# mushroomfire/mdapy

Hardware: AMD Instinct MI355X
Metric: atoms/sec for neighbor+CNA on 10M-atom FCC Cu; 1/2/4/8-GPU scaling (higher is better)
Workload: dtype f64 (CNA pair tests: f32 filter + f64 finish, labels exact); 1 GPU; FCC Cu a=3.615, 136^3 cells per GPU (10061824 atoms/GPU, 10061824 total), build_neighbor(rc=0.854a=3.08721, max_neigh=16) + fixed-cutoff CNA as one C-ABI call (mdh_build_neighbor_fcna: lists and labels), positions resident in HBM; atoms_per_gpu=10061824, max_neigh=16, parallelism=single, world_size_checked=1, launched_by=single process

## Files before the change

### mdapy_amd/csrc/cna_core.hpp

```cpp
#pragma once
#include "common.hpp"

namespace mdh {

struct Rows {
    uint64_t w0, w1, w2, w3;
    __device__ __forceinline__ unsigned row(int a) const
    {
        const uint64_t w = (a < 8) ? ((a < 4) ? w0 : w1) : ((a < 12) ? w2 : w3);
        return (unsigned)(w >> ((a & 3) << 4)) & 0xffffu;
    }
};

template <int NN>
__device__ __forceinline__ Rows pack_rows(const unsigned (&adj)[NN])
{
    Rows r{0, 0, 0, 0};
#pragma unroll
    for (int a = 0; a < NN; ++a) {
        const uint64_t v = (uint64_t)adj[a] << ((a & 3) << 4);
        if (a < 4) r.w0 |= v;
        else if (a < 8) r.w1 |= v;
        else if (a < 12) r.w2 |= v;
        else r.w3 |= v;
    }
    return r;
}

struct RowsLds {
    const unsigned short *base;
    int stride;
    __device__ __forceinline__ unsigned row(int a) const { return base[a * stride]; }
};
template <int NN>
__device__ __forceinline__ RowsLds spill_rows(const Rows &R, unsigned short *base, int stride)
{
#pragma unroll
    for (int a = 0; a < NN; ++a) base[a * stride] = (unsigned short)R.row(a);
    return RowsLds{base, stride};
}

template <int NN>
struct RowsReg {
    unsigned v[NN];
    __device__ __forceinline__ explicit RowsReg(const unsigned (&adj)[NN])
    {
#pragma unroll
        for (int k = 0; k < NN; ++k) v[k] = adj[k];
    }
    __device__ __forceinline__ unsigned row(int a) const
    {
        unsigned r = v[0];
#pragma unroll
        for (int k = 1; k < NN; ++k) {
            unsigned t = v[k];
            asm("" : "+v"(t));
            r = (a == k) ? t : r;
        }
        return r;
    }
};

template <class RT>
__device__ __forceinline__ void signature(const RT &R, int ni, unsigned limit_mask, int &ncn, int &nb, int &chain)
{
    const unsigned common = R.row(ni);
    ncn = __popc(common);
    const unsigned pool = common & limit_mask;
    int bonds = 0, maxdeg = 0;
    for (unsigned m = pool; m; m &= m - 1) {
        const int deg = __popc(R.row(__ffs(m) - 1) & pool);
        bonds += deg;
        maxdeg = deg > maxdeg ? deg : maxdeg;
    }
    nb = bonds >> 1;
    if (nb <= 1) { chain = nb; return; }
    if (nb == 2) { chain = maxdeg == 2 ? 2 : 1; return; }
    const int npool = __popc(pool);
    if (nb == npool && (npool == 4 || npool == 5)) { chain = nb; return; }
    int best = 0;
    unsigned left = pool;
    while (left) {
        unsigned comp = left & (0u - left), frontier = comp;
        while (frontier) {
            const int a = __ffs(frontier) - 1;
            frontier &= frontier - 1;
            const unsigned grow = R.row(a) & pool & ~comp;
            comp |= grow;
            frontier |= grow;
        }
        int cb = 0;
        for (unsigned m = comp; m; m &= m - 1)
            cb += __popc(R.row(__ffs(m) - 1) & comp);
        cb >>= 1;
        best = cb > best ? cb : best;
        left &= ~comp;
    }
    chain = best;
}

__device__ __forceinline__ double fold(double d, double L, double t_zero, double t_one)
{
    const double shift = (d >= t_one) ? L : ((d >= t_zero) ? 0.0 : -L);
    return d - shift;
}

template <int NN>
__device__ __forceinline__ int span_class(const DBox &b, const double (&p)[NN], int axis)
{
    double mn = p[0], mx = p[0];
#pragma unroll
    for (int a = 1; a < NN; ++a) {
        mn = fmin(mn, p[a]);
        mx = fmax(mx, p[a]);
    }
    const double span = mx - mn;
    const double lim = fmin(b.tn[axis][3], -b.tn[axis][0]);
    const double zero = fmin(b.tn[axis][2], -b.tn[axis][1]);
    if (!(span < lim))
        return 0;
    return span < zero ? 2 : 1;
}

template <bool TRI, int NN>
__device__ __forceinline__ Rows bond_rows_reg(const DBox &b, const double (&px)[NN], const double (&py)[NN],
                                              const double (&pz)[NN], double cut2)
{
    unsigned adj[NN];
#pragma unroll
    for (int a = 0; a < NN; ++a)
        adj[a] = 0;
#pragma unroll
    for (int a = 0; a < NN; ++a)
#pragma unroll
        for (int c = a + 1; c < NN; ++c) {
            const double d2 = pair_d2<TRI>(b, px[a], py[a], pz[a], px[c], py[c], pz[c]);
            if (d2 <= cut2) {
                adj[a] |= 1u << c;
                adj[c] |= 1u << a;
            }
        }
    return pack_rows<NN>(adj);
}

template <int NN>
__device__ __forceinline__ Rows bond_rows_ortho(const DBox &b, const double (&px)[NN], const double (&py)[NN],
                                                const double (&pz)[NN], double cut2, bool plain)
{
    unsigned adj[NN];
#pragma unroll
    for (int a = 0; a < NN; ++a)
        adj[a] = 0;
    if (plain) {
#pragma unroll
        for (int a = 0; a < NN; ++a)
#pragma unroll
            for (int c = a + 1; c < NN; ++c) {
                const double dx = px[c] - px[a], dy = py[c] - py[a], dz = pz[c] - pz[a];
                if (dx * dx + dy * dy + dz * dz <= cut2) {
                    adj[a] |= 1u << c;
                    adj[c] |= 1u << a;
                }
            }
        return pack_rows<NN>(adj);
    }
#pragma unroll
    for (int a = 0; a < NN; ++a)
#pragma unroll
        for (int c = a + 1; c < NN; ++c) {
            double dx = px[c] - px[a], dy = py[c] - py[a], dz = pz[c] - pz[a];
            if (b.pbc[0]) dx = fold(dx, b.h[0], b.tn[0][1], b.tn[0][2]);
            if (b.pbc[1]) dy = fold(dy, b.h[4], b.tn[1][1], b.tn[1][2]);
            if (b.pbc[2]) dz = fold(dz, b.h[8], b.tn[2][1], b.tn[2][2]);
            const double d2 = dx * dx + dy * dy + dz * dz;
            if (d2 <= cut2) {
                adj[a] |= 1u << c;
                adj[c] |= 1u << a;
            }
        }
    return pack_rows<NN>(adj);
}

template <int NN>
__device__ __forceinline__ int span_class3(const DBox &b, const double (&px)[NN], const double (&py)[NN], const double (&pz)[NN])
{
    int cls = 2;
    if (b.pbc[0]) cls = min(cls, span_class<NN>(b, px, 0));
    if (b.pbc[1]) cls = min(cls, span_class<NN>(b, py, 1));
    if (b.pbc[2]) cls = min(cls, span_class<NN>(b, pz, 2));
    return cls;
}

template <int NN, class RT>
__device__ __forceinline__ int fcna_label(const RT &R)
{
    int n421 = 0, n422 = 0, n555 = 0, n444 = 0, n666 = 0;
    for (int ni = 0; ni < NN; ++ni) {
        int ncn, nb, ch;
        signature(R, ni, (1u << NN) - 1u, ncn, nb, ch);
        if (ncn == 4 && nb == 2) { n421 += (ch == 1); n422 += (ch == 2); }
        else if (ncn == 5 && nb == 5 && ch == 5) ++n555;
        else if (ncn == 4 && nb == 4 && ch == 4) ++n444;
        else if (ncn == 6 && nb == 6 && ch == 6) ++n666;
    }
    if (n421 == 12) return 1;
    if (n421 == 6 && n422 == 6) return 2;
    if (n555 == 12) return 4;
    if (n666 == 8 && n444 == 6) return 3;
    return 0;
}

template <int NW>
__device__ __forceinline__ bool six_bonds_one_cluster(const unsigned (&P)[NW], unsigned common, unsigned bonded)
{
    unsigned reach = bonded & (0u - bonded);
#pragma unroll
    for (int it = 0; it < 5; ++it) {
        unsigned acc = 0;
#pragma unroll
        for (int k = 0; k < NW; ++k) {
            const unsigned lo = (unsigned)(((int)(reach << (31 - 2 * k))) >> 31) & 0xffffu;
            const unsigned hi = (unsigned)(((int)(reach << (30 - 2 * k))) >> 31) & 0xffff0000u;
            acc |= P[k] & (lo | hi);
        }
        reach |= (acc | (acc >> 16)) & common & 0xffffu;
    }
    return (bonded & ~reach) == 0u;
}
struct CnaCounts { int n421, n422, n555, n444, n666; };
template <int NN, int MAXO = NN, class RT = RowsLds>
__device__ __forceinline__ CnaCounts cna_counts_words(const unsigned (&adj)[NN], const RT &L)
{
    constexpr int NW = (NN + 1) / 2;
    unsigned P[NW];
#pragma unroll
    for (int k = 0; k < NW; ++k) P[k] = adj[2 * k] | ((2 * k + 1 < NN) ? (adj[2 * k + 1] << 16) : 0u);
    unsigned packed = 0;
#pragma unroll
    for (int ni = 0; ni < NN; ++ni) {
        if (MAXO < NN && (packed >> 20) > (unsigned)MAXO)
            continue;
        const unsigned common = adj[ni];
        const unsigned ncn = (unsigned)__popc(common);
        const unsigned c2 = common | (common << 16);
        unsigned twice = 0, touched = 0;
#pragma unroll
        for (int k = 0; k < NW; ++k) {
            const unsigned lo = (unsigned)(((int)(common << (31 - 2 * k))) >> 31) & 0xffffu;
            const unsigned hi = (unsigned)(((int)(common << (30 - 2 * k))) >> 31) & 0xffff0000u;
            const unsigned xk = P[k] & c2 & (lo | hi);
            twice += __popc(xk);
            touched |= xk;
        }
        const unsigned key = ncn + (twice << 4);
        const unsigned three = (__popc((touched | (touched >> 16)) & 0xffffu) == 3) ? 1u << 4 : 1u;
        unsigned inc = 1u << 20;
        inc = key == 68u ? three : inc;
        inc = key == 165u ? 1u << 8 : inc;
        inc = key == 132u ? 1u << 12 : inc;
        if (key == 198u)
            inc = six_bonds_one_cluster<NW>(P, common, (touched | (touched >> 16)) & 0xffffu) ? 1u << 16 : 1u << 20;
        packed += inc;
    }
    return CnaCounts{(int)(packed & 15u), (int)((packed >> 4) & 15u), (int)((packed >> 8) & 15u), (int)((packed >> 12) & 15u), (int)((packed >> 16) & 15u)};
}
template <int NN, class RT = RowsLds>
__device__ __forceinline__ int fcna_label_words(const unsigned (&adj)[NN], const RT &L)
{
    const CnaCounts c = cna_counts_words<NN, NN - 12, RT>(adj, L);
    if (c.n421 == 12) return 1;
    if (c.n421 == 6 && c.n422 == 6) return 2;
    if (c.n555 == 12) return 4;
    if (c.n666 == 8 && c.n444 == 6) return 3;
    return 0;
}

template <int NN> constexpr int pair_a(int p) { int a = 0; while (p >= NN - 1 - a) { p -= NN - 1 - a; ++a; } return a; }
template <int NN> constexpr int pair_c(int p) { int a = 0; while (p >= NN - 1 - a) { p -= NN - 1 - a; ++a; } return a + 1 + p; }
template <int NN, int NV, int P>
__device__ __forceinline__ void pair_tests_f32(const float (&ux)[NV], const float (&uy)[NV], const float (&uz)[NV], float negc,
                                               unsigned (&adj)[NN], unsigned &w)
{
    constexpr int NP = NN * (NN - 1) / 2;
    if constexpr (P + 1 < NP) {
        constexpr int a0 = pair_a<NN>(P), c0 = pair_c<NN>(P), a1 = pair_a<NN>(P + 1), c1 = pair_c<NN>(P + 1);
        float t0, t1, t2, s0, s1, s2;
#define MDH_PAIR2_HEAD                                                                                                                 \
            "v_sub_f32 %[t0], %[xc], %[xa]\n\t"                                                                                        \
            "v_sub_f32 %[t1], %[yc], %[ya]\n\t"                                                                                        \
            "v_sub_f32 %[t2], %[zc], %[za]\n\t"                                                                                        \
            "v_sub_f32 %[s0], %[xd], %[xb]\n\t"                                                                                        \
            "v_sub_f32 %[s1], %[yd], %[yb]\n\t"                                                                                        \
            "v_sub_f32 %[s2], %[zd], %[zb]\n\t"                                                                                        \
            "v_fma_f32 %[t0], %[t0], %[t0], %[negc]\n\t"                                                                               \
            "v_fma_f32 %[s0], %[s0], %[s0], %[negc]\n\t"                                                                               \
            "v_fmac_f32 %[t0], %[t1], %[t1]\n\t"                                                                                       \
            "v_fmac_f32 %[s0], %[s1], %[s1]\n\t"                                                                                       \
            "v_fmac_f32 %[t0], %[t2], %[t2]\n\t"                                                                                       \
            "v_fmac_f32 %[s0], %[s2], %[s2]\n\t"                                                                                       \
            "v_min3_u32 %[w], %[w], %[t0], %[s0]\n\t"                                                                                  \
            "v_lshrrev_b32 %[t0], 31, %[t0]\n\t"                                                                                       \
            "v_lshrrev_b32 %[s0], 31, %[s0]\n\t"
#define MDH_PAIR2_IN                                                                                                                   \
            [xc] "v"(ux[c0]), [xa] "v"(ux[a0]), [yc] "v"(uy[c0]), [ya] "v"(uy[a0]), [zc] "v"(uz[c0]), [za] "v"(uz[a0]),                 \
            [xd] "v"(ux[c1]), [xb] "v"(ux[a1]), [yd] "v"(uy[c1]), [yb] "v"(uy[a1]), [zd] "v"(uz[c1]), [zb] "v"(uz[a1]),                 \
            [negc] "v"(negc), [sc] "n"(c0), [sa] "n"(a0), [sd] "n"(c1), [sb] "n"(a1)
        if constexpr (a0 == a1) {
            asm(MDH_PAIR2_HEAD
                "v_lshl_or_b32 %[ra], %[t0], %[sc], %[ra]\n\t"
                "v_lshl_or_b32 %[rc], %[t0], %[sa], %[rc]\n\t"
                "v_lshl_or_b32 %[ra], %[s0], %[sd], %[ra]\n\t"
                "v_lshl_or_b32 %[rd], %[s0], %[sb], %[rd]"
                : [t0] "=&v"(t0), [t1] "=&v"(t1), [t2] "=&v"(t2), [s0] "=&v"(s0), [s1] "=&v"(s1), [s2] "=&v"(s2), [w] "+v"(w),
                  [ra] "+v"(adj[a0]), [rc] "+v"(adj[c0]), [rd] "+v"(adj[c1])
                : MDH_PAIR2_IN);
        } else if constexpr (c0 == c1) {
            asm(MDH_PAIR2_HEAD
                "v_lshl_or_b32 %[ra], %[t0], %[sc], %[ra]\n\t"
                "v_lshl_or_b32 %[rc], %[t0], %[sa], %[rc]\n\t"
                "v_lshl_or_b32 %[rb], %[s0], %[sd], %[rb]\n\t"
                "v_lshl_or_b32 %[rc], %[s0], %[sb], %[rc]"
                : [t0] "=&v"(t0), [t1] "=&v"(t1), [t2] "=&v"(t2), [s0] "=&v"(s0), [s1] "=&v"(s1), [s2] "=&v"(s2), [w] "+v"(w),
                  [ra] "+v"(adj[a0]), [rc] "+v"(adj[c0]), [rb] "+v"(adj[a1])
                : MDH_PAIR2_IN);
        } else {
            static_assert(a0 != c1 && c0 != a1, "two pairs of a block share a row that the block binds twice");
            asm(MDH_PAIR2_HEAD
                "v_lshl_or_b32 %[ra], %[t0], %[sc], %[ra]\n\t"
                "v_lshl_or_b32 %[rc], %[t0], %[sa], %[rc]\n\t"
                "v_lshl_or_b32 %[rb], %[s0], %[sd], %[rb]\n\t"
                "v_lshl_or_b32 %[rd], %[s0], %[sb], %[rd]"
                : [t0] "=&v"(t0), [t1] "=&v"(t1), [t2] "=&v"(t2), [s0] "=&v"(s0), [s1] "=&v"(s1), [s2] "=&v"(s2), [w] "+v"(w),
                  [ra] "+v"(adj[a0]), [rc] "+v"(adj[c0]), [rb] "+v"(adj[a1]), [rd] "+v"(adj[c1])
                : MDH_PAIR2_IN);
        }
#undef MDH_PAIR2_HEAD
#undef MDH_PAIR2_IN
        pair_tests_f32<NN, NV, P + 2>(ux, uy, uz, negc, adj, w);
    } else if constexpr (P < NP) {
        constexpr int a = pair_a<NN>(P), c = pair_c<NN>(P);
        float t0, t1, t2;
        asm("v_sub_f32 %[t0], %[xc], %[xa]\n\t"
            "v_sub_f32 %[t1], %[yc], %[ya]\n\t"
            "v_sub_f32 %[t2], %[zc], %[za]\n\t"
            "v_fma_f32 %[t0], %[t0], %[t0], %[negc]\n\t"
            "v_fmac_f32 %[t0], %[t1], %[t1]\n\t"
            "v_fmac_f32 %[t0], %[t2], %[t2]\n\t"
            "v_min_u32 %[w], %[w], %[t0]\n\t"
            "v_lshrrev_b32 %[t0], 31, %[t0]\n\t"
            "v_lshl_or_b32 %[ra], %[t0], %[sc], %[ra]\n\t"
            "v_lshl_or_b32 %[rc], %[t0], %[sa], %[rc]"
            : [t0] "=&v"(t0), [t1] "=&v"(t1), [t2] "=&v"(t2), [w] "+v"(w), [ra] "+v"(adj[a]), [rc] "+v"(adj[c])
            : [xc] "v"(ux[c]), [xa] "v"(ux[a]), [yc] "v"(uy[c]), [ya] "v"(uy[a]), [zc] "v"(uz[c]), [za] "v"(uz[a]), [negc] "v"(negc),
              [sc] "n"(c), [sa] "n"(a));
    }
}

__device__ __forceinline__ void defer(int *__restrict__ todo, int64_t i) { todo[1 + atomicAdd(&todo[0], 1)] = (int)i; }

}
```

### mdapy_amd/csrc/neighbor_lane.hip

```cpp
#include "common.hpp"
#include "grid.hpp"
#include "cna_core.hpp"
#include <algorithm>
#include <cmath>
#include <type_traits>
#include <cstdio>
#include <cstdlib>
#include <cstring>
#include <mutex>
#include <vector>

namespace mdh {
namespace lane {

constexpr int cen_cap(int nw) { return 80 * nw; }
__host__ __device__ constexpr int ticket_row(int M, bool cna_rows) { return (cna_rows && ((M + 4) & ~3) < 28) ? 28 : ((M + 4) & ~3); }
static constexpr int NEUTRAL = img::CELL_NEUTRAL;
static constexpr int NEUTRAL3 = img::NEUTRAL;

struct FastDiv {
    unsigned mul, sh1, sh2, d;
    __device__ __forceinline__ unsigned div(unsigned n) const
    {
        const unsigned t = __umulhi(mul, n);
        return (t + ((n - t) >> sh1)) >> sh2;
    }
};
static FastDiv make_fastdiv(unsigned d)
{
    FastDiv f{0, 0, 0, d};
    unsigned l = 0;
    while ((1ull << l) < d) ++l;
    f.mul = (unsigned)(((1ull << 32) * ((1ull << l) - d)) / d + 1);
    f.sh1 = l < 1 ? l : 1;
    f.sh2 = l > 1 ? l - 1 : 0;
    return f;
}
struct Shape { int txy, tz; FastDiv by_nt2, by_nt1; unsigned mhz, mhxy; };
static Shape make_shape(int txy, int tz, int nt1, int nt2)
{
    return Shape{txy, tz, make_fastdiv((unsigned)nt2), make_fastdiv((unsigned)nt1), (65536u + (unsigned)tz + 1u) / ((unsigned)tz + 2u),
                 (65536u + (unsigned)txy + 1u) / ((unsigned)txy + 2u)};
}
typedef __attribute__((address_space(3))) unsigned char lds_byte;
typedef int Int4 __attribute__((ext_vector_type(4)));

static int g_last_plan[8];
static int g_last_listed = -1;
#ifdef MDH_STAMPS
__device__ unsigned long long g_stamps[65536 * 8];
#define STAMP(k) do { if (tid == 0 && !parent && tile.id < 65536) g_stamps[tile.id * 8 + (k)] = __builtin_amdgcn_s_memtime(); } while (0)
#else
#define STAMP(k) do {} while (0)
#endif

__device__ __forceinline__ void lds_barrier()
{
    asm volatile("s_waitcnt lgkmcnt(0)\n\ts_barrier" ::: "memory");
}

template <int NW>
__device__ __forceinline__ int excl_scan_block(int v, int *scratch, int *total)
{
    const int lane = threadIdx.x & 63, w = threadIdx.x >> 6;
    int inc = v;
#pragma unroll
    for (int d = 1; d < 64; d <<= 1) {
        int t = __shfl_up(inc, d, 64);
        if (lane >= d) inc += t;
    }
    if (lane == 63) scratch[w] = inc;
    __syncthreads();
    int off = 0, tot = 0;
#pragma unroll
    for (int k = 0; k < NW; ++k) {
        if (k < w) off += scratch[k];
        tot += scratch[k];
    }
    *total = tot;
    return off + inc - v;
}

__device__ __forceinline__ int combine_codes(int cc, int ca) { return img::combine(cc, ca); }

template <int KIND>
__device__ __forceinline__ double exact_d2(const DBox &b, double xj, double yj, double zj, double xi, double yi, double zi,
                                           int code)
{
    double dx = xj - xi, dy = yj - yi, dz = zj - zi;
    if (KIND == 1) {
        dx = dx - b.h[0] * (double)img::axis(code, 0);
        dy = dy - b.h[4] * (double)img::axis(code, 1);
        dz = dz - b.h[8] * (double)img::axis(code, 2);
    }
    if (KIND == 2)
        pbc<true>(b, dx, dy, dz);
    return dx * dx + dy * dy + dz * dz;
}

#define MDH_CAND2(X1, Y1, Z1, X2, Y2, Z2)                                                                                            \
    "v_sub_f32 v116, " X1 ", %[sx]\n\t"                                                                                              \
    "v_sub_f32 v119, " X2 ", %[sx]\n\t"                                                                                              \
    "v_sub_f32 v117, " Y1 ", %[sy]\n\t"                                                                                              \
    "v_sub_f32 v120, " Y2 ", %[sy]\n\t"                                                                                              \
    "v_sub_f32 v118, " Z1 ", %[sz]\n\t"                                                                                              \
    "v_sub_f32 v121, " Z2 ", %[sz]\n\t"                                                                                              \
    "v_fma_f32 v116, v116, v116, %[negc]\n\t"                                                                                        \
    "v_fma_f32 v119, v119, v119, %[negc]\n\t"                                                                                        \
    "v_fmac_f32 v116, v117, v117\n\t"                                                                                                \
    "v_fmac_f32 v119, v120, v120\n\t"                                                                                                \
    "v_fmac_f32 v116, v118, v118\n\t"                                                                                                \
    "v_fmac_f32 v119, v121, v121\n\t"                                                                                                \
    "v_alignbit_b32 %[m], %[m], v116, 31\n\t"                                                                                        \
    "v_alignbit_b32 %[m], %[m], v119, 31\n\t"                                                                                        \
    "v_min3_u32 %[w], %[w], v116, v119\n\t"
__device__ __forceinline__ void scan_run_asm(unsigned a, int rem, float sx, float sy, float sz, float negc, unsigned &mask,
                                             unsigned &w)
{
    unsigned long long save;
    unsigned m;
    asm volatile("s_mov_b64 %[save], exec\n\t"
                 "v_mov_b32 %[m], 0\n"
                 ".Lscan_top_%=:\n\t"
                 "v_cmp_lt_i32 vcc, 0, %[rem]\n\t"
                 "s_and_b64 exec, exec, vcc\n\t"
                 "s_cbranch_execz .Lscan_end_%=\n\t"
                 "ds_read_b128 v[100:103], %[a]\n\t"
                 "ds_read_b128 v[104:107], %[a] offset:16\n\t"
                 "ds_read_b128 v[108:111], %[a] offset:32\n\t"
                 "ds_read_b128 v[112:115], %[a] offset:48\n\t"
                 "v_add_u32 %[a], 64, %[a]\n\t"
                 "v_add_u32 %[rem], -4, %[rem]\n\t"
                 "s_waitcnt lgkmcnt(2)\n\t" MDH_CAND2("v100", "v101", "v102", "v104", "v105", "v106")
                 "s_waitcnt lgkmcnt(0)\n\t" MDH_CAND2("v108", "v109", "v110", "v112", "v113", "v114")
                 "s_branch .Lscan_top_%=\n"
                 ".Lscan_end_%=:\n\t"
                 "s_mov_b64 exec, %[save]\n\t"
                 : [m] "=&v"(m), [w] "+v"(w), [a] "+v"(a), [rem] "+v"(rem), [save] "=&s"(save)
                 : [sx] "v"(sx), [sy] "v"(sy), [sz] "v"(sz), [negc] "v"(negc)
                 : "vcc", "scc", "memory", "v100", "v101", "v102", "v103", "v104", "v105", "v106", "v107", "v108", "v109", "v110",
                   "v111", "v112", "v113", "v114", "v115", "v116", "v117", "v118", "v119", "v120", "v121");
    mask = m;
}
__device__ __forceinline__ void scan_run12_asm(unsigned a, float sx, float sy, float sz, float negc, unsigned &mask, unsigned &w)
{
    unsigned m;
    asm volatile("v_mov_b32 %[m], 0\n\t"
                 "ds_read_b128 v[100:103], %[a]\n\t"
                 "ds_read_b128 v[104:107], %[a] offset:16\n\t"
                 "ds_read_b128 v[108:111], %[a] offset:32\n\t"
                 "ds_read_b128 v[112:115], %[a] offset:48\n\t"
                 "s_waitcnt lgkmcnt(2)\n\t" MDH_CAND2("v100", "v101", "v102", "v104", "v105", "v106")
                 "ds_read_b128 v[100:103], %[a] offset:64\n\t"
                 "ds_read_b128 v[104:107], %[a] offset:80\n\t"
                 "s_waitcnt lgkmcnt(2)\n\t" MDH_CAND2("v108", "v109", "v110", "v112", "v113", "v114")
                 "ds_read_b128 v[108:111], %[a] offset:96\n\t"
                 "ds_read_b128 v[112:115], %[a] offset:112\n\t"
                 "s_waitcnt lgkmcnt(2)\n\t" MDH_CAND2("v100", "v101", "v102", "v104", "v105", "v106")
                 "ds_read_b128 v[100:103], %[a] offset:128\n\t"
                 "ds_read_b128 v[104:107], %[a] offset:144\n\t"
                 "s_waitcnt lgkmcnt(2)\n\t" MDH_CAND2("v108", "v109", "v110", "v112", "v113", "v114")
                 "ds_read_b128 v[108:111], %[a] offset:160\n\t"
                 "ds_read_b128 v[112:115], %[a] offset:176\n\t"
                 "s_waitcnt lgkmcnt(2)\n\t" MDH_CAND2("v100", "v101", "v102", "v104", "v105", "v106")
                 "s_waitcnt lgkmcnt(0)\n\t" MDH_CAND2("v108", "v109", "v110", "v112", "v113", "v114")
                 : [m] "=&v"(m), [w] "+v"(w)
                 : [a] "v"(a), [sx] "v"(sx), [sy] "v"(sy), [sz] "v"(sz), [negc] "v"(negc)
                 : "memory", "v100", "v101", "v102", "v103", "v104", "v105", "v106", "v107", "v108", "v109", "v110", "v111", "v112", "v113",
                   "v114", "v115", "v116", "v117", "v118", "v119", "v120", "v121");
    mask = m;
}
#undef MDH_CAND2
__device__ __forceinline__ int run_slots(int len)
{
    return (len + 3) & ~3;
}

__device__ __forceinline__ bool sqrt_fast_ok(double x)
{
    return x >= 0x1p-767 && x < 0x1p+1000;
}
__device__ __forceinline__ double sqrt_fast(double x)
{
    const double y = __builtin_amdgcn_rsq(x);
    double g = x * y;
    double h = y * 0.5;
    const double r = __builtin_fma(-h, g, 0.5);
    g = __builtin_fma(g, r, g);
    h = __builtin_fma(h, r, h);
    const double d0 = __builtin_fma(-g, g, x);
    g = __builtin_fma(d0, h, g);
    const double d1 = __builtin_fma(-g, g, x);
    return __builtin_fma(d1, h, g);
}

template <bool SELF, bool TRI>
__device__ __forceinline__ unsigned scan_run_f64(const double2 *__restrict__ lxy, const double *__restrict__ lz,
                                                 const unsigned short *__restrict__ lsh, const DBox &b, double rcsq, int k0, int len,
                                                 int li, double xi, double yi, double zi)
{
    unsigned m = 0;
    const int S = run_slots(len);
    for (int j = 0; j < S; ++j) {
        const int k = k0 + j;
        bool h = false;
        if (j < len) {
            const double2 cj = lxy[k];
            const double d2 = exact_d2<TRI ? 2 : 1>(b, cj.x, cj.y, lz[k], xi, yi, zi, TRI ? 0 : lsh[k]);
            h = (d2 <= rcsq) && (!SELF || k != li);
        }
        m = m + m + (h ? 1u : 0u);
    }
    return m;
}

template <bool TRI, int NN, class Index>
__device__ __forceinline__ int lane_fcna(const DBox &b, Index index_of, const double2 *__restrict__ lxy,
                                         const double *__restrict__ lz, bool plain, double cut2)
{
    double px[NN], py[NN], pz[NN];
#pragma unroll
    for (int a = 0; a < NN; ++a) {
        const int k = index_of(a);
        const double2 c = lxy[k];
        px[a] = c.x; py[a] = c.y; pz[a] = lz[k];
    }
    Rows R;
    if (TRI) {
        R = bond_rows_reg<true, NN>(b, px, py, pz, cut2);
    } else {
        const int cls = plain ? 2 : span_class3<NN>(b, px, py, pz);
        if (cls == 0)
            return -1;
        R = bond_rows_ortho<NN>(b, px, py, pz, cut2, cls == 2);
    }
    return fcna_label<NN>(R);
}

template <int NN, class Index>
__device__ __forceinline__ int lane_fcna_f32(Index index_of, const float4 *__restrict__ f4, float negc, float W)
{
    float ux[NN], uy[NN], uz[NN];
#pragma unroll
    for (int a = 0; a < NN; ++a) {
        const float4 c = f4[index_of(a)];
        ux[a] = c.x; uy[a] = c.y; uz[a] = c.z;
    }
    unsigned adj[NN];
#pragma unroll
    for (int a = 0; a < NN; ++a)
        adj[a] = 0;
    unsigned w = 0x7f7fffffu;
    pair_tests_f32<NN, NN, 0>(ux, uy, uz, negc, adj, w);
    if (w <= __float_as_uint(W))
        return -1;
    return fcna_label_words<NN, RowsReg<NN>>(adj, RowsReg<NN>(adj));
}

__device__ __forceinline__ int bit_select(int m, int a, int b)
{
    int d;
    asm("v_bfi_b32 %0, %1, %2, %3" : "=v"(d) : "v"(m), "v"(a), "v"(b));
    return d;
}
__device__ __forceinline__ void quad_transpose(int (&P)[4][4], int odd1, int odd2)
{
#pragma unroll
    for (int pp = 0; pp < 4; pp += 2)
#pragma unroll
        for (int w = 0; w < 4; ++w) {
            const int x = bit_select(odd1, P[pp][w], P[pp + 1][w]);
            const int y = __builtin_amdgcn_mov_dpp(x, 0xB1, 0xF, 0xF, true);
            P[pp + 1][w] = bit_select(odd1, P[pp + 1][w], y);
            P[pp][w] = bit_select(odd1, y, P[pp][w]);
        }
#pragma unroll
    for (int pp = 0; pp < 2; ++pp)
#pragma unroll
        for (int w = 0; w < 4; ++w) {
            const int x = bit_select(odd2, P[pp][w], P[pp + 2][w]);
            const int y = __builtin_amdgcn_mov_dpp(x, 0x4E, 0xF, 0xF, true);
            P[pp + 2][w] = bit_select(odd2, P[pp + 2][w], y);
            P[pp][w] = bit_select(odd2, y, P[pp][w]);
        }
}

struct IndirectSrc { const double *x, *y, *z; const unsigned short *mv; const int *order; };
__device__ __forceinline__ CellGrid::Packed load_atom(const IndirectSrc &src, int id, int coded)
{
    int code = (int)img::ATOM_NEUTRAL;
    if (coded) code = src.mv[id];
    return CellGrid::Packed{src.x[id], src.y[id], src.z[id], id, code};
}
struct __attribute__((packed, aligned(4))) Ids4 { int v[4]; };
template <bool IND>
__device__ __forceinline__ CellGrid::Packed load_record(const CellGrid::Packed *__restrict__ pk, const IndirectSrc &src, int q, int coded)
{
    if (!IND)
        return pk[q];
    return load_atom(src, src.order[q], coded);
}

template <bool COUNT, bool TRI, bool LOOP, bool FCNA, bool TK8, int NW = 4, bool IND = false>
#ifdef MDH_FCNA_F64
#define MDH_FCNA_LEAN false
#else
#define MDH_FCNA_LEAN true
#endif
__global__ __launch_bounds__(NW * 64, (TK8 && (!FCNA || (MDH_FCNA_LEAN && !LOOP))) ? 16 / NW : 1) void k_neighbor_lane(
    const CellGrid::Packed *__restrict__ pk, const int *__restrict__ cell_start, DBox b,
    Grid g, double rc, float negc, float W, int *__restrict__ verlet, double *__restrict__ dist, int *__restrict__ nn,
    int M, int write_pads, int cap, int *__restrict__ flags, unsigned char *__restrict__ tile_flag, int nt0,
    int nt1, int nt2, Shape ts, const int *__restrict__ tile_list, const int *__restrict__ n_live, int list_mode,
    int *__restrict__ max_count, int *__restrict__ flagged, const int *__restrict__ parent, int parent_nt2, int nsub,
    int flag_slot, int *__restrict__ pattern, int *__restrict__ cna_todo, int jt0, int rw, int tile_base, int *__restrict__ listed_sink,
    int cen_lo, int cen_hi, IndirectSrc isrc)
{
    const int TXY = ts.txy, TZ = ts.tz;
    const int coded = IND ? flags[4] : 0;
    const int HXY = TXY + 2, HZ = TZ + 2, NH = HXY * HXY * HZ;
    constexpr int CENC = cen_cap(NW);

    extern __shared__ __attribute__((aligned(16))) unsigned char smem[];
    const int tid = threadIdx.x, lane = tid & 63;
    typedef typename std::conditional<TK8, unsigned char, unsigned short>::type Ticket;
    constexpr int JB = TK8 ? 5 : 8;
    float4 *f4 = reinterpret_cast<float4 *>(smem);
    double2 *lxy = reinterpret_cast<double2 *>(f4 + cap);
    double *lz = reinterpret_cast<double *>(lxy + cap);
    unsigned *cen = reinterpret_cast<unsigned *>(lz + cap);
    unsigned short *lsh = reinterpret_cast<unsigned short *>(cen + CENC);
    Ticket *tk = reinterpret_cast<Ticket *>(lsh + cap + (cap & 1));
    const unsigned f4_lds = (unsigned)(unsigned long)(lds_byte *)smem;
    const int TKS = ticket_row(M, false);
    const int wstride = max(rw * TKS, 256 / (int)sizeof(Ticket));
    auto hc = [&](int t) -> unsigned & { return reinterpret_cast<unsigned *>(tk + (size_t)(t >> 6) * wstride)[t & 63]; };
    __shared__ unsigned hr[NW * 64 + 2];
    __shared__ int scan_tmp[NW];
    __shared__ int s_flag[4];

    const double rcsq = rc * rc, pad = rc + 1.0;
    const double cw = rc;
    int vmax = 0;

    const int nlive = parent ? min(*n_live, nt0 * nt1 * parent_nt2) * nsub : ((list_mode && tile_list) ? *n_live : nt0 * nt1 * nt2);
    const int per = (nlive + 7) / 8;
    if (parent && listed_sink && blockIdx.x == 0 && tid == 0)
        *listed_sink = min(*n_live, nt0 * nt1 * parent_nt2);
    struct Tile { int id, T0, T1, T2; bool empty; };
    struct Halo { int cnt, src, img, hz; bool edge, centre; };
    auto tile_of = [&](int slot) {
        Tile t;
        int t0, t1, t2;
        if (parent) {
            const int pt = parent[slot / nsub];
            t2 = (pt % parent_nt2) * nsub + slot % nsub;
            t1 = (pt / parent_nt2) % nt1;
            t0 = pt / (parent_nt2 * nt1);
            t.id = (t0 * nt1 + t1) * nt2 + t2;
        } else {
            t.id = (list_mode && tile_list) ? tile_list[slot] : slot + tile_base;
            const unsigned col = ts.by_nt2.div((unsigned)t.id);
            t2 = t.id - (int)col * nt2;
            t0 = (int)ts.by_nt1.div(col);
            t1 = (int)col - t0 * nt1;
        }
        t.T0 = t0 * TXY; t.T1 = t1 * TXY; t.T2 = t2 * TZ;
        t.empty = t.T2 >= g.nc[2];
        return t;
    };
    auto halo_of = [&](const Tile &t) {
        Halo h{0, 0, NEUTRAL, 0, false, false};
        if (tid < NH && !t.empty) {
            const int hcol = (int)(((unsigned)tid * ts.mhz) >> 16);
            h.hz = tid - hcol * HZ;
            const int hx = (int)(((unsigned)hcol * ts.mhxy) >> 16), hy = hcol - hx * HXY;
            const int g0 = t.T0 + hx - 1, g1 = t.T1 + hy - 1, g2 = t.T2 + h.hz - 1;
            const bool in0 = b.pbc[0] ? (g0 >= -1 && g0 <= g.nc[0]) : (g0 >= 0 && g0 < g.nc[0]);
            const bool in1 = b.pbc[1] ? (g1 >= -1 && g1 <= g.nc[1]) : (g1 >= 0 && g1 < g.nc[1]);
            const bool in2 = b.pbc[2] ? (g2 >= -1 && g2 <= g.nc[2]) : (g2 >= 0 && g2 < g.nc[2]);
            if (in0 && in1 && in2) {
                const int a0 = g0 < 0 ? g0 + g.nc[0] : (g0 >= g.nc[0] ? g0 - g.nc[0] : g0);
                const int a1 = g1 < 0 ? g1 + g.nc[1] : (g1 >= g.nc[1] ? g1 - g.nc[1] : g1);
                const int a2 = g2 < 0 ? g2 + g.nc[2] : (g2 >= g.nc[2] ? g2 - g.nc[2] : g2);
                const int c = (a0 * g.nc[1] + a1) * g.nc[2] + a2;
                h.src = cell_start[c];
                h.cnt = cell_start[c + 1] - h.src;
                const int n0 = g0 < 0 ? 1 : (g0 >= g.nc[0] ? -1 : 0);
                const int n1 = g1 < 0 ? 1 : (g1 >= g.nc[1] ? -1 : 0);
                const int n2 = g2 < 0 ? 1 : (g2 >= g.nc[2] ? -1 : 0);
                h.img = (n0 + 1) | ((n1 + 1) << 2) | ((n2 + 1) << 4);
                h.edge = (!b.pbc[0] && (a0 == 0 || a0 == g.nc[0] - 1)) || (!b.pbc[1] && (a1 == 0 || a1 == g.nc[1] - 1)) ||
                         (!b.pbc[2] && (a2 == 0 || a2 == g.nc[2] - 1));
                h.centre = hx >= 1 && hx <= TXY && hy >= 1 && hy <= TXY && h.hz >= 1 && h.hz <= TZ && g0 < g.nc[0] && g1 < g.nc[1] && g2 < g.nc[2] &&
                           g0 >= cen_lo && g0 < cen_hi;
            }
        }
        return h;
    };
    auto request = [&](const Halo &h, double (&ra)[4], double (&rb)[4], double (&rc4)[4], int (&rd)[4], int (&rm)[4]) {
        Ids4 ids{};
        if (IND) ids = *reinterpret_cast<const Ids4 *>(isrc.order + h.src);
#pragma unroll
        for (int v = 0; v < 4; ++v) {
            const int q = h.cnt > 0 ? h.src + min(v, h.cnt - 1) : 0;
            const CellGrid::Packed a = IND ? load_atom(isrc, v < h.cnt ? ids.v[v] : (h.cnt > 0 ? ids.v[0] : 0), coded) : load_record<false>(pk, isrc, q, coded);
            ra[v] = a.x; rb[v] = a.y; rc4[v] = a.z; rd[v] = a.id; rm[v] = a.code;
        }
    };
    for (int jt = jt0 + (int)(blockIdx.x >> 3); jt < per; jt += (int)(gridDim.x >> 3)) {
        const int slot = (int)(blockIdx.x & 7) * per + jt;
        if (slot >= nlive)
            break;
        const Tile tile = tile_of(slot);
        STAMP(0);
        Halo cur = halo_of(tile);
#ifdef MDH_STAMPS
        asm volatile("" : "+v"(cur.src), "+v"(cur.cnt));
        STAMP(1);
#endif
        double pa[4], pb[4], pc[4];
        int pd[4], pm[4];
        request(cur, pa, pb, pc, pd, pm);
        if (flags[0] != 0)
            return;
        const int tile_id = tile.id, T0 = tile.T0, T1 = tile.T1, T2 = tile.T2;
        const int cnt = cur.cnt, src = cur.src, img = cur.img, hz = cur.hz;
        const bool edge = cur.edge, centre_cell = cur.centre;
        if (tid == 0) { s_flag[0] = 0; s_flag[1] = 0; s_flag[2] = 0; s_flag[3] = 0; }
        hc(tid) = (unsigned)cnt;

        int total2;
        const int off2 = excl_scan_block<NW>(cnt | (centre_cell ? cnt << 16 : 0), scan_tmp, &total2);
        const int total = total2 & 0xffff, ncentres = total2 >> 16;
        const int off0 = off2 & 0xffff, coff = off2 >> 16;
        bool ok = !(total > cap || ncentres > CENC);
        const bool no_centres = ncentres == 0;
        if (no_centres) ok = false;
        STAMP(2);
        if (ok && tid < NH && hz >= 1 && hz <= HZ - 2) {
            const unsigned k0 = (unsigned)off0 - hc(tid - 1), len = hc(tid - 1) + (unsigned)cnt + hc(tid + 1);
            hr[tid] = k0 | (len << 16);
            if (len > (TK8 ? 32u : 96u)) s_flag[2] = 1;
            if (TK8 && len > 12u) s_flag[3] = 1;
        }
        if (ok && cnt > 0) {
            double X0, Y0, Z0, XS, YS, ZS;
            const int code0 = combine_codes(img, img::ATOM_NEUTRAL);
            if (TRI) {
                const double f0 = (double)(T0 - 1) * (cw / b.thick[0]) + (double)img::axis(code0, 0);
                const double f1 = (double)(T1 - 1) * (cw / b.thick[1]) + (double)img::axis(code0, 1);
                const double f2 = (double)(T2 - 1) * (cw / b.thick[2]) + (double)img::axis(code0, 2);
                XS = b.o[0] + f0 * b.h[0] + f1 * b.h[3] + f2 * b.h[6];
                YS = b.o[1] + f0 * b.h[1] + f1 * b.h[4] + f2 * b.h[7];
                ZS = b.o[2] + f0 * b.h[2] + f1 * b.h[5] + f2 * b.h[8];
                X0 = XS; Y0 = YS; Z0 = ZS;
            } else {
                X0 = b.o[0] + (double)(T0 - 1) * cw; Y0 = b.o[1] + (double)(T1 - 1) * cw; Z0 = b.o[2] + (double)(T2 - 1) * cw;
                XS = X0 + b.h[0] * (double)img::axis(code0, 0); YS = Y0 + b.h[4] * (double)img::axis(code0, 1);
                ZS = Z0 + b.h[8] * (double)img::axis(code0, 2);
            }
            const float flo = (float)(-1.5 * cw);
            const float fhx = (float)(((double)HXY + 1.5) * cw), fhz = (float)(((double)HZ + 1.5) * cw);
            bool general = code0 != NEUTRAL3, far = false;
            auto stage4 = [&](int k, const double (&a)[4], const double (&bb)[4], const double (&c)[4], const int (&d)[4], const int (&m)[4]) {
#pragma unroll
                for (int v = 0; v < 4; ++v) {
                    if (k + v < cnt) {
                        int code = code0;
                        float ux, uy, uz;
                        if (TRI) {
                            double wx = a[v], wy = bb[v], wz = c[v];
                            wrap<true>(b, wx, wy, wz);
                            const double rx = wx - XS, ry = wy - YS, rz = wz - ZS;
                            ux = (float)rx; uy = (float)ry; uz = (float)rz;
                            if (edge) {
                                const double s0 = (rx * b.hi[0] + ry * b.hi[3] + rz * b.hi[6]) * (b.thick[0] / cw);
                                const double s1 = (rx * b.hi[1] + ry * b.hi[4] + rz * b.hi[7]) * (b.thick[1] / cw);
                                const double s2 = (rx * b.hi[2] + ry * b.hi[5] + rz * b.hi[8]) * (b.thick[2] / cw);
                                far = far || !(s0 >= -1.5 && s0 <= (double)HXY + 1.5 && s1 >= -1.5 && s1 <= (double)HXY + 1.5 && s2 >= -1.5 && s2 <= (double)HZ + 1.5);
                            }
                        } else {
                            ux = (float)(a[v] - XS); uy = (float)(bb[v] - YS); uz = (float)(c[v] - ZS);
                        }
                        if (!TRI && m[v] != img::ATOM_NEUTRAL) {
                            code = combine_codes(img, m[v]);
                            ux = (float)((a[v] - b.h[0] * (double)img::axis(code, 0)) - X0);
                            uy = (float)((bb[v] - b.h[4] * (double)img::axis(code, 1)) - Y0);
                            uz = (float)((c[v] - b.h[8] * (double)img::axis(code, 2)) - Z0);
                            general = true;
                        }
                        if (!TRI && edge)
                            far = far || !(ux >= flo && ux <= fhx && uy >= flo && uy <= fhx && uz >= flo && uz <= fhz);
                        const int p = off0 + k + v;
#ifdef MDH_EXP_GATHER
                        f4[p] = make_float4(ux, uy, uz, __int_as_float(src + k + v));
#else
                        f4[p] = make_float4(ux, uy, uz, __int_as_float(d[v]));
#endif
                        lxy[p] = make_double2(a[v], bb[v]);
                        lz[p] = c[v];
                        lsh[p] = (unsigned short)code;
                        if (centre_cell) cen[coff + k + v] = (unsigned)p | ((unsigned)tid << 11);
                    }
                }
            };
            if (TK8) {
                for (int k = 0; k < cnt; k += 4) {
                    double a[4], bb[4], c[4];
                    int d[4], m[4];
#pragma unroll
                    for (int v = 0; v < 4; ++v) {
                        if (k == 0) { a[v] = pa[v]; bb[v] = pb[v]; c[v] = pc[v]; d[v] = pd[v]; m[v] = pm[v]; }
                        else {
                            const int q = src + min(k + v, cnt - 1);
                            const CellGrid::Packed r = load_record<IND>(pk, isrc, q, coded);
                            a[v] = r.x; bb[v] = r.y; c[v] = r.z; d[v] = r.id; m[v] = r.code;
                        }
                    }
                    stage4(k, a, bb, c, d, m);
                }
            } else {
                double a[4], bb[4], c[4];
                int d[4], m[4];
#pragma unroll
                for (int v = 0; v < 4; ++v) { a[v] = pa[v]; bb[v] = pb[v]; c[v] = pc[v]; d[v] = pd[v]; m[v] = pm[v]; }
                for (int k = 0; k < cnt; k += 4) {
                    double na[4], nb[4], nc[4];
                    int nd[4], nm[4];
#pragma unroll
                    for (int v = 0; v < 4; ++v) {
                        const int q = src + min(k + 4 + v, cnt - 1);
                        const CellGrid::Packed r = load_record<IND>(pk, isrc, q, coded);
                        na[v] = r.x; nb[v] = r.y; nc[v] = r.z; nd[v] = r.id; nm[v] = r.code;
                    }
                    stage4(k, a, bb, c, d, m);
#pragma unroll
                    for (int v = 0; v < 4; ++v) { a[v] = na[v]; bb[v] = nb[v]; c[v] = nc[v]; d[v] = nd[v]; m[v] = nm[v]; }
                }
            }
            if (general) s_flag[0] = 1;
            if (far) s_flag[1] = 1;
        }
        __syncthreads();
        STAMP(3);
        if (ok && (s_flag[1] | s_flag[2]))
            ok = false;
        if (!ok && !no_centres && tid == 0) {
            if (tile_flag) tile_flag[tile_id] = 1;
            flagged[atomicAdd(&flags[flag_slot], 1)] = tile_id;
        }
        const bool general_tile = s_flag[0] != 0;
        const bool short_runs = TK8 && s_flag[3] == 0;
        const int wv = tid >> 6;
        Ticket *tkw = tk + (size_t)wv * wstride;
        const int A2 = HXY * HZ;
        auto run_cell = [&](int cbv, int r) {
            const int r3 = (r * 11) >> 5;
            return cbv + __mul24(r3, A2 - 3 * HZ) + __mul24(r, HZ) - (A2 + HZ);
// ... 812 lines not shown
```

Before: 7.137 billion atoms/s.

## Add FCC certificate fast path and pairwise CNA labeling for 12-neighbour atoms

Rewrites the f32 pair tests to process two pairs per asm block and build adjacency rows with alignbit shifts, which produces bit-reversed rows that are then flipped. For 12-neighbour atoms it first checks an FCC certificate (every row has four bonds and each bonded pair shares exactly two common neighbours) and returns the FCC label directly. Otherwise it falls back to a new pairwise common-neighbour accumulation that decides FCC/HCP/ICO labels without the per-neighbour bond-chain loop. It also tweaks the generic word-based counter to keep the 0xffff mask in a register. The aim is to cut the VALU work in the CNA classification of the dominant FCC case, at the cost of more inline asm (including v_bitop3) and new label logic that must exactly match the old classifier.

```diff
diff --git a/mdapy_amd/csrc/cna_core.hpp b/mdapy_amd/csrc/cna_core.hpp
--- a/mdapy_amd/csrc/cna_core.hpp
+++ b/mdapy_amd/csrc/cna_core.hpp
@@ -236,6 +236,8 @@
 #pragma unroll
     for (int k = 0; k < NW; ++k) P[k] = adj[2 * k] | ((2 * k + 1 < NN) ? (adj[2 * k + 1] << 16) : 0u);
     unsigned packed = 0;
+    unsigned lo16 = 0xffffu;
+    asm("" : "+v"(lo16));
 #pragma unroll
     for (int ni = 0; ni < NN; ++ni) {
         if (MAXO < NN && (packed >> 20) > (unsigned)MAXO)
@@ -246,9 +248,9 @@
         unsigned twice = 0, touched = 0;
 #pragma unroll
         for (int k = 0; k < NW; ++k) {
-            const unsigned lo = (unsigned)(((int)(common << (31 - 2 * k))) >> 31) & 0xffffu;
-            const unsigned hi = (unsigned)(((int)(common << (30 - 2 * k))) >> 31) & 0xffff0000u;
-            const unsigned xk = P[k] & c2 & (lo | hi);
+            const unsigned lo = (unsigned)(((int)(common << (31 - 2 * k))) >> 31);
+            const unsigned hi = (unsigned)(((int)(common << (30 - 2 * k))) >> 31);
+            const unsigned xk = P[k] & c2 & ((lo & lo16) | (hi & ~lo16));
             twice += __popc(xk);
             touched |= xk;
         }
@@ -356,6 +358,142 @@
     }
 }
 
+template <int NN, int NV, int P>
+__device__ __forceinline__ void pair_tests_f32_rev(const float (&ux)[NV], const float (&uy)[NV], const float (&uz)[NV], float negc,
+                                                   unsigned (&adj)[NN], unsigned &w)
+{
+    constexpr int NP = NN * (NN - 1) / 2;
+    if constexpr (P + 1 < NP) {
+        constexpr int a0 = pair_a<NN>(P), c0 = pair_c<NN>(P), a1 = pair_a<NN>(P + 1), c1 = pair_c<NN>(P + 1);
+        if constexpr (a0 > 0 && c0 == a0 + 1) adj[a0] <<= 1;
+        if constexpr (a1 > 0 && c1 == a1 + 1) adj[a1] <<= 1;
+        float t0, t1, t2, s0, s1, s2;
+#define MDH_PAIR2_HEAD                                                                                                                 \
+            "v_sub_f32 %[t0], %[xc], %[xa]\n\t"                                                                                        \
+            "v_sub_f32 %[t1], %[yc], %[ya]\n\t"                                                                                        \
+            "v_sub_f32 %[t2], %[zc], %[za]\n\t"                                                                                        \
+            "v_sub_f32 %[s0], %[xd], %[xb]\n\t"                                                                                        \
+            "v_sub_f32 %[s1], %[yd], %[yb]\n\t"                                                                                        \
+            "v_sub_f32 %[s2], %[zd], %[zb]\n\t"                                                                                        \
+            "v_fma_f32 %[t0], %[t0], %[t0], %[negc]\n\t"                                                                               \
+            "v_fma_f32 %[s0], %[s0], %[s0], %[negc]\n\t"                                                                               \
+            "v_fmac_f32 %[t0], %[t1], %[t1]\n\t"                                                                                       \
+            "v_fmac_f32 %[s0], %[s1], %[s1]\n\t"                                                                                       \
+            "v_fmac_f32 %[t0], %[t2], %[t2]\n\t"                                                                                       \
+            "v_fmac_f32 %[s0], %[s2], %[s2]\n\t"                                                                                       \
+            "v_min3_u32 %[w], %[w], %[t0], %[s0]\n\t"
+#define MDH_PAIR2_IN                                                                                                                   \
+            [xc] "v"(ux[c0]), [xa] "v"(ux[a0]), [yc] "v"(uy[c0]), [ya] "v"(uy[a0]), [zc] "v"(uz[c0]), [za] "v"(uz[a0]),                 \
+            [xd] "v"(ux[c1]), [xb] "v"(ux[a1]), [yd] "v"(uy[c1]), [yb] "v"(uy[a1]), [zd] "v"(uz[c1]), [zb] "v"(uz[a1]),                 \
+            [negc] "v"(negc)
+        if constexpr (a0 == a1) {
+            asm(MDH_PAIR2_HEAD
+                "v_alignbit_b32 %[ra], %[ra], %[t0], 31\n\t"
+                "v_alignbit_b32 %[rc], %[rc], %[t0], 31\n\t"
+                "v_alignbit_b32 %[ra], %[ra], %[s0], 31\n\t"
+                "v_alignbit_b32 %[rd], %[rd], %[s0], 31"
+                : [t0] "=&v"(t0), [t1] "=&v"(t1), [t2] "=&v"(t2), [s0] "=&v"(s0), [s1] "=&v"(s1), [s2] "=&v"(s2), [w] "+v"(w),
+                  [ra] "+v"(adj[a0]), [rc] "+v"(adj[c0]), [rd] "+v"(adj[c1])
+                : MDH_PAIR2_IN);
+        } else if constexpr (c0 == c1) {
+            asm(MDH_PAIR2_HEAD
+                "v_alignbit_b32 %[ra], %[ra], %[t0], 31\n\t"
+                "v_alignbit_b32 %[rc], %[rc], %[t0], 31\n\t"
+                "v_alignbit_b32 %[rb], %[rb], %[s0], 31\n\t"
+                "v_alignbit_b32 %[rc], %[rc], %[s0], 31"
+                : [t0] "=&v"(t0), [t1] "=&v"(t1), [t2] "=&v"(t2), [s0] "=&v"(s0), [s1] "=&v"(s1), [s2] "=&v"(s2), [w] "+v"(w),
+                  [ra] "+v"(adj[a0]), [rc] "+v"(adj[c0]), [rb] "+v"(adj[a1])
+                : MDH_PAIR2_IN);
+        } else {
+            static_assert(a0 != c1 && c0 != a1, "two pairs of a block share a row that the block binds twice");
+            asm(MDH_PAIR2_HEAD
+                "v_alignbit_b32 %[ra], %[ra], %[t0], 31\n\t"
+                "v_alignbit_b32 %[rc], %[rc], %[t0], 31\n\t"
+                "v_alignbit_b32 %[rb], %[rb], %[s0], 31\n\t"
+                "v_alignbit_b32 %[rd], %[rd], %[s0], 31"
+                : [t0] "=&v"(t0), [t1] "=&v"(t1), [t2] "=&v"(t2), [s0] "=&v"(s0), [s1] "=&v"(s1), [s2] "=&v"(s2), [w] "+v"(w),
+                  [ra] "+v"(adj[a0]), [rc] "+v"(adj[c0]), [rb] "+v"(adj[a1]), [rd] "+v"(adj[c1])
+                : MDH_PAIR2_IN);
+        }
+#undef MDH_PAIR2_HEAD
+#undef MDH_PAIR2_IN
+        pair_tests_f32_rev<NN, NV, P + 2>(ux, uy, uz, negc, adj, w);
+    } else {
+        if constexpr (P < NP) {
+            constexpr int a = pair_a<NN>(P), c = pair_c<NN>(P);
+            if constexpr (a > 0 && c == a + 1) adj[a] <<= 1;
+            float t0, t1, t2;
+            asm("v_sub_f32 %[t0], %[xc], %[xa]\n\t"
+                "v_sub_f32 %[t1], %[yc], %[ya]\n\t"
+                "v_sub_f32 %[t2], %[zc], %[za]\n\t"
+                "v_fma_f32 %[t0], %[t0], %[t0], %[negc]\n\t"
+                "v_fmac_f32 %[t0], %[t1], %[t1]\n\t"
+                "v_fmac_f32 %[t0], %[t2], %[t2]\n\t"
+                "v_min_u32 %[w], %[w], %[t0]\n\t"
+                "v_alignbit_b32 %[ra], %[ra], %[t0], 31\n\t"
+                "v_alignbit_b32 %[rc], %[rc], %[t0], 31"
+                : [t0] "=&v"(t0), [t1] "=&v"(t1), [t2] "=&v"(t2), [w] "+v"(w), [ra] "+v"(adj[a]), [rc] "+v"(adj[c])
+                : [xc] "v"(ux[c]), [xa] "v"(ux[a]), [yc] "v"(uy[c]), [ya] "v"(uy[a]), [zc] "v"(uz[c]), [za] "v"(uz[a]), [negc] "v"(negc));
+        }
+        adj[NN - 1] <<= 1;
+    }
+}
+
+template <int NN>
+__device__ __forceinline__ bool fcc_certificate(const unsigned (&r)[NN])
+{
+    unsigned bad = 0;
+#pragma unroll
+    for (int a = 0; a < NN; ++a)
+        bad |= (unsigned)__popc(r[a]) - 4u;
+#pragma unroll
+    for (int a = 0; a < NN; ++a)
+#pragma unroll
+        for (int c = a + 1; c < NN; ++c) {
+            unsigned m, x;
+            asm("v_bfe_i32 %[m], %[ra], %[c], 1\n\t"
+                "v_bitop3_b32 %[x], %[ra], %[rc], %[m] bitop3:0x80\n\t"
+                "v_bcnt_u32_b32 %[x], %[x], %[m]\n\t"
+                "v_or_b32 %[bad], %[bad], %[x]"
+                : [m] "=&v"(m), [x] "=&v"(x), [bad] "+v"(bad)
+                : [ra] "v"(r[a]), [rc] "v"(r[c]), [c] "n"(c));
+        }
+    return bad == 0u;
+}
+
+template <int NN>
+__device__ __forceinline__ int fcna_label_pairs(const unsigned (&r)[NN])
+{
+    static_assert(NN == 12, "fcna_label_pairs decides the labels of 12-neighbour atoms only");
+    unsigned acc[NN];
+#pragma unroll
+    for (int a = 0; a < NN; ++a) acc[a] = 0;
+#pragma unroll
+    for (int a = 0; a < NN; ++a)
+#pragma unroll
+        for (int c = a + 1; c < NN; ++c) {
+            unsigned m, x;
+            asm("v_bfe_i32 %[m], %[ra], %[c], 1\n\t"
+                "v_bitop3_b32 %[x], %[ra], %[rc], %[m] bitop3:0x80\n\t"
+                "v_bcnt_u32_b32 %[aa], %[x], %[aa]\n\t"
+                "v_bcnt_u32_b32 %[ac], %[x], %[ac]\n\t"
+                "v_lshl_or_b32 %[aa], %[x], 16, %[aa]\n\t"
+                "v_lshl_or_b32 %[ac], %[x], 16, %[ac]"
+                : [m] "=&v"(m), [x] "=&v"(x), [aa] "+v"(acc[a]), [ac] "+v"(acc[c])
+                : [ra] "v"(r[a]), [rc] "v"(r[c]), [c] "n"(c));
+        }
+    unsigned bad4 = 0, bad5 = 0, sum_touched = 0;
+#pragma unroll
+    for (int a = 0; a < NN; ++a) {
+        const unsigned key = (unsigned)__popc(r[a]) + ((acc[a] & 0xffffu) << 4);
+        bad4 |= key ^ 68u;
+        bad5 |= key ^ 165u;
+        sum_touched += (unsigned)__popc(acc[a] >> 16);
+    }
+    if (bad4 == 0u) return sum_touched == 48u ? 1 : (sum_touched == 42u ? 2 : 0);
+    return bad5 == 0u ? 4 : 0;
+}
+
 __device__ __forceinline__ void defer(int *__restrict__ todo, int64_t i) { todo[1 + atomicAdd(&todo[0], 1)] = (int)i; }
 
 }
diff --git a/mdapy_amd/csrc/neighbor_lane.hip b/mdapy_amd/csrc/neighbor_lane.hip
--- a/mdapy_amd/csrc/neighbor_lane.hip
+++ b/mdapy_amd/csrc/neighbor_lane.hip
@@ -251,10 +251,19 @@
     for (int a = 0; a < NN; ++a)
         adj[a] = 0;
     unsigned w = 0x7f7fffffu;
-    pair_tests_f32<NN, NN, 0>(ux, uy, uz, negc, adj, w);
+    pair_tests_f32_rev<NN, NN, 0>(ux, uy, uz, negc, adj, w);
+    unsigned r[NN];
+#pragma unroll
+    for (int a = 0; a < NN; ++a)
+        r[a] = adj[NN - 1 - a];
     if (w <= __float_as_uint(W))
         return -1;
-    return fcna_label_words<NN, RowsReg<NN>>(adj, RowsReg<NN>(adj));
+    if constexpr (NN == 12) {
+        if (fcc_certificate<NN>(r))
+            return 1;
+        return fcna_label_pairs<NN>(r);
+    }
+    return fcna_label_words<NN, RowsReg<NN>>(r, RowsReg<NN>(r));
 }
 
 __device__ __forceinline__ int bit_select(int m, int a, int b)
```

Measured after the change: 7.525 billion atoms/s, median of 6. 1.05x the previous value.
